# excamera/alfalfa

Measured on AMD Instinct MI355X. Metric: 1080p macroblocks/s decode (bit-exact vs reference), higher is better.
Workload: dtype u8

## Files before the change

### alfalfa_amd/csrc/parse_common.hh

```
#pragma once
#include <stddef.h>
#include <stdint.h>

#include "../../include/alfalfa_amd.h"
#include "vp8_tables.h"

#if defined( __HIPCC__ )
#define AA_HD __host__ __device__
#else
#define AA_HD
#endif

namespace aa {

enum MbMode : uint8_t { DC_PRED, V_PRED, H_PRED, TM_PRED, B_PRED, NEARESTMV, NEARMV, ZEROMV, NEWMV, SPLITMV };
enum BMode : uint8_t { B_DC_PRED, B_TM_PRED, B_VE_PRED, B_HE_PRED, B_LD_PRED, B_RD_PRED, B_VR_PRED, B_VL_PRED,
                       B_HD_PRED, B_HU_PRED, LEFT4X4, ABOVE4X4, ZERO4X4, NEW4X4 };
enum RefFrame : uint8_t { CURRENT_FRAME, LAST_FRAME, GOLDEN_FRAME, ALTREF_FRAME };
enum BlockType { Y_AFTER_Y2 = 0, Y2 = 1, UV = 2, Y_WITHOUT_Y2 = 3 };

constexpr int8_t kKfYModeTree[8] = { -B_PRED, 2, 4, 6, -DC_PRED, -V_PRED, -H_PRED, -TM_PRED };
constexpr int8_t kYModeTree[8] = { -DC_PRED, 2, 4, 6, -V_PRED, -H_PRED, -TM_PRED, -B_PRED };
constexpr int8_t kUvModeTree[6] = { -DC_PRED, 2, -V_PRED, 4, -H_PRED, -TM_PRED };
constexpr int8_t kBModeTree[18] = { -B_DC_PRED, 2, -B_TM_PRED, 4, -B_VE_PRED, 6, 8, 12, -B_HE_PRED, 10,
                                    -B_RD_PRED, -B_VR_PRED, -B_LD_PRED, 14, -B_VL_PRED, 16, -B_HD_PRED, -B_HU_PRED };
constexpr int8_t kSmallMvTree[14] = { 2, 8, 4, 6, -0, -1, -2, -3, 10, 12, -4, -5, -6, -7 };
constexpr int8_t kMvRefTree[8] = { -ZEROMV, 2, -NEARESTMV, 4, -NEARMV, 6, -NEWMV, -SPLITMV };
constexpr int8_t kSubMvRefTree[6] = { -LEFT4X4, 2, -ABOVE4X4, 4, -ZERO4X4, -NEW4X4 };
constexpr int8_t kSplitMvTree[6] = { -3, 2, -2, 4, -0, -1 };
constexpr int8_t kSegmentIdTree[6] = { 2, 4, -0, -1, -2, -3 };

constexpr uint8_t kZigzag[16] = { 0, 1, 4, 8, 5, 2, 3, 6, 9, 12, 13, 10, 7, 11, 14, 15 };
constexpr uint8_t kBand[17] = { 0, 1, 2, 3, 6, 4, 5, 6, 6, 6, 6, 6, 6, 6, 6, 7, 0 };

constexpr uint8_t kSplitLayout[4][16] = { { 0, 0, 0, 0, 0, 0, 0, 0, 1, 1, 1, 1, 1, 1, 1, 1 },
                                          { 0, 0, 1, 1, 0, 0, 1, 1, 0, 0, 1, 1, 0, 0, 1, 1 },
                                          { 0, 0, 1, 1, 0, 0, 1, 1, 2, 2, 3, 3, 2, 2, 3, 3 },
                                          { 0, 1, 2, 3, 4, 5, 6, 7, 8, 9, 10, 11, 12, 13, 14, 15 } };
constexpr uint8_t kSplitFirst[4][16] = { { 0, 8 }, { 0, 2 }, { 0, 2, 8, 10 }, { 0, 1, 2, 3, 4, 5, 6, 7, 8, 9, 10, 11, 12, 13, 14, 15 } };
constexpr uint8_t kSplitCount[4] = { 2, 2, 4, 16 };

struct CoeffProbs { uint8_t coeff_probs[4][8][3][11]; };
struct HeaderParams {
  uint32_t first_off, first_size;
  uint32_t bd_bitpos;
  uint8_t bd_range, bd_active;
  uint8_t key, nparts;
  uint32_t part_off[8], part_size[8];
  uint16_t mbw, mbh;
  uint8_t seg_enabled, seg_update_map, seg_tree_probs[3];
  uint8_t skip_enabled, prob_skip, prob_inter, prob_last, prob_golden;
  uint8_t sign_bias_golden, sign_bias_alt;
  uint8_t loop_filter_level, fadj_enabled;
  int8_t fadj_ref[4], fadj_mode[4];
  int16_t seg_level[4];
  uint8_t y_mode_probs[4], uv_mode_probs[3], mv_probs[2][19];
  uint8_t pad[3];
};
struct FrameParams : CoeffProbs, HeaderParams {};
static_assert( sizeof( FrameParams ) % 4 == 0 && sizeof( HeaderParams ) % 4 == 0 && sizeof( FrameParams ) == sizeof( CoeffProbs ) + sizeof( HeaderParams ),
               "FrameParams / HeaderParams are copied as words" );

struct HeaderTables {
  int8_t kf_y_mode_tree[8], y_mode_tree[8], uv_mode_tree[6], b_mode_tree[18], small_mv_tree[14], mv_ref_tree[8], sub_mv_ref_tree[6], split_mv_tree[6], segment_id_tree[6];
  uint8_t kf_y_mode_probs[4], kf_uv_mode_probs[3], b_mode_probs[9], mv_counts_to_probs[24], split_mv_probs[3], submv_ref_probs[15];
  uint8_t split_layout[4][16], split_first[4][16], split_count[4];
  uint8_t kf_b_mode_probs[900];
  uint8_t pad[2];
};
static_assert( sizeof( HeaderTables ) % 4 == 0, "HeaderTables is copied as words" );
constexpr HeaderTables make_header_tables()
{
  HeaderTables t {};
  for ( int i = 0; i < 8; i++ ) { t.kf_y_mode_tree[i] = kKfYModeTree[i]; t.y_mode_tree[i] = kYModeTree[i]; t.mv_ref_tree[i] = kMvRefTree[i]; }
  for ( int i = 0; i < 6; i++ ) { t.uv_mode_tree[i] = kUvModeTree[i]; t.sub_mv_ref_tree[i] = kSubMvRefTree[i]; t.split_mv_tree[i] = kSplitMvTree[i]; t.segment_id_tree[i] = kSegmentIdTree[i]; }
  for ( int i = 0; i < 18; i++ ) t.b_mode_tree[i] = kBModeTree[i];
  for ( int i = 0; i < 14; i++ ) t.small_mv_tree[i] = kSmallMvTree[i];
  for ( int i = 0; i < 4; i++ ) t.kf_y_mode_probs[i] = k_kf_y_mode_probs[i];
  for ( int i = 0; i < 3; i++ ) { t.kf_uv_mode_probs[i] = k_kf_uv_mode_probs[i]; t.split_mv_probs[i] = k_split_mv_probs[i]; }
  for ( int i = 0; i < 9; i++ ) t.b_mode_probs[i] = k_b_mode_probs[i];
  for ( int i = 0; i < 24; i++ ) t.mv_counts_to_probs[i] = k_mv_counts_to_probs[i];
  for ( int i = 0; i < 15; i++ ) t.submv_ref_probs[i] = k_submv_ref_probs[i];
  for ( int i = 0; i < 4; i++ ) { t.split_count[i] = kSplitCount[i]; for ( int j = 0; j < 16; j++ ) { t.split_layout[i][j] = kSplitLayout[i][j]; t.split_first[i][j] = kSplitFirst[i][j]; } }
  for ( int i = 0; i < 900; i++ ) t.kf_b_mode_probs[i] = k_kf_b_mode_probs[i];
  return t;
}
constexpr HeaderTables kHeaderTables = make_header_tables();



struct BoolState { uint32_t bitpos; uint8_t range, active; };

class BoolReader32
{
  const uint8_t * base_ = nullptr;
  uint32_t pos_ = 0, end_ = 0;
  uint32_t value_ = 0;
  int count_ = 0;
  uint32_t range_ = 255;
  uint32_t cache_ = 0;
  uint32_t cache_n_ = 0;

  AA_HD inline uint32_t next_byte()
  {
    if ( cache_n_ == 0 ) {
      if ( pos_ < end_ ) {
        const uintptr_t a = reinterpret_cast<uintptr_t>( base_ + pos_ );
        const uint32_t skip = static_cast<uint32_t>( a & 3u );
        cache_ = *reinterpret_cast<const uint32_t *>( a - skip ) >> ( 8u * skip );
        cache_n_ = 4u - skip;
      } else { cache_ = 0; cache_n_ = 4u; }
    }
    const uint32_t byte = pos_ < end_ ? ( cache_ & 0xFFu ) : 0u;
    cache_ >>= 8; cache_n_--; pos_++;
    return byte;
  }

public:
  AA_HD BoolReader32() {}
  AA_HD void resume( const uint8_t * base, uint32_t size, const BoolState & st )
  {
    base_ = base; end_ = size; range_ = st.range;
    const uint32_t byte = st.bitpos >> 3, r = st.bitpos & 7;
    pos_ = byte; cache_n_ = 0;
    uint32_t b = 0;
    for ( int k = 0; k < 3; k++ ) b = ( b << 8 ) | next_byte();
    value_ = ( static_cast<uint32_t>( st.active ) << 24 ) | ( ( b << r ) & 0xFFFFFFu );
    count_ = 24 - static_cast<int>( r );
  }
  AA_HD void reset( const uint8_t * base, uint32_t size )
  {
    BoolState st; st.bitpos = 8; st.range = 255; st.active = size ? base[0] : 0;
    resume( base, size, st );
  }
  AA_HD inline int get( const uint32_t prob )
  {
    const uint32_t split = 1 + ( ( ( range_ - 1 ) * prob ) >> 8 );
    if ( count_ < 0 ) {
      value_ |= next_byte() << ( 16 - count_ );
      count_ += 8;
    }
    const uint32_t bigsplit = split << 24;
    int bit;
    uint32_t range;
    if ( value_ >= bigsplit ) { range = range_ - split; value_ -= bigsplit; bit = 1; }
    else { range = split; bit = 0; }
    const int shift = __builtin_clz( range ) - 24;
    range_ = range << shift;
    value_ <<= shift;
    count_ -= shift;
    return bit;
  }
  AA_HD inline int flag() { return get( 128 ); }
  AA_HD inline int literal( int bits ) { int v = 0; while ( bits-- ) v = ( v << 1 ) | get( 128 ); return v; }
  AA_HD inline int tree( const int8_t * nodes, const uint8_t * probs )
  {
    int i = 0;
    while ( ( i = nodes[i + get( probs[i >> 1] )] ) > 0 ) {}
    return -i;
  }
};

struct Mv {
  int16_t x = 0, y = 0;
  AA_HD bool zero() const { return x == 0 && y == 0; }
  AA_HD bool operator==( const Mv & o ) const { return x == o.x && y == o.y; }
};

AA_HD inline int clamp_int( int v, int lo, int hi ) { return v < lo ? lo : ( v > hi ? hi : v ); }

template <class BD>
AA_HD inline int16_t read_mv_component( BD & bd, const uint8_t * p, const HeaderTables & T )
{
  enum { MV_IS_SHORT, SIGN, SHORT, BITS = SHORT + 8 - 1, MV_LONG_BITS = 10 };
  int x = 0;
  if ( bd.get( p[MV_IS_SHORT] ) ) {
    for ( int i = 0; i < 3; i++ ) x += bd.get( p[BITS + i] ) << i;
    for ( int i = MV_LONG_BITS - 1; i > 3; i-- ) x += bd.get( p[BITS + i] ) << i;
    if ( !( x & 0xFFF0 ) || bd.get( p[BITS + 3] ) ) x += 8;
  } else {
    x = bd.tree( T.small_mv_tree, p + SHORT );
  }
  x <<= 1;
  if ( x && bd.get( p[SIGN] ) ) x = -x;
  return static_cast<int16_t>( x );
}

template <class BD>
AA_HD inline Mv read_mv( BD & bd, const HeaderParams & fp, const HeaderTables & T )
{
  Mv m;
  m.y = read_mv_component( bd, fp.mv_probs[0], T );
  m.x = read_mv_component( bd, fp.mv_probs[1], T );
  return m;
}

AA_HD inline Mv clamp_mv( Mv m, unsigned col, unsigned row, unsigned mbw, unsigned mbh )
{
  const int to_left = clamp_int( -( static_cast<int>( col * 16 ) << 3 ) - 128, -32768, 32767 );
  const int to_right = clamp_int( ( static_cast<int>( ( mbw - 1 - col ) * 16 ) << 3 ) + 128, -32768, 32767 );
  const int to_top = clamp_int( -( static_cast<int>( row * 16 ) << 3 ) - 128, -32768, 32767 );
  const int to_bottom = clamp_int( ( static_cast<int>( ( mbh - 1 - row ) * 16 ) << 3 ) + 128, -32768, 32767 );
  m.x = static_cast<int16_t>( clamp_int( m.x, to_left, to_right ) );
  m.y = static_cast<int16_t>( clamp_int( m.y, to_top, to_bottom ) );
  return m;
}

AA_HD inline uint8_t mb_lf_level( const HeaderParams & fp, unsigned segment_id, unsigned ref_frame, unsigned y_mode )
{
  if ( !fp.loop_filter_level ) return 0;
  int level = fp.seg_level[segment_id];
  if ( fp.fadj_enabled ) {
    level += fp.fadj_ref[ref_frame];
    if ( ref_frame == CURRENT_FRAME ) level += ( y_mode == B_PRED ) ? fp.fadj_mode[0] : 0;
    else if ( y_mode == ZEROMV ) level += fp.fadj_mode[1];
    else if ( y_mode == SPLITMV ) level += fp.fadj_mode[3];
    else level += fp.fadj_mode[2];
  }
  return static_cast<uint8_t>( level <= 0 ? 0 : ( level > 63 ? 63 : level ) );
}

AA_HD inline void segment_fixup( const HeaderParams & fp, aa_mb_info & mb, uint8_t & map )
{
  if ( fp.seg_update_map ) map = mb.segment_id;
  else {
    mb.segment_id = map;
    mb.lf_level = mb_lf_level( fp, map, mb.ref_frame, mb.y_mode );
  }
}

AA_HD inline bool mv_flipped( const HeaderParams & fp, unsigned ref_frame )
{
  return ( ref_frame == GOLDEN_FRAME && fp.sign_bias_golden ) || ( ref_frame == ALTREF_FRAME && fp.sign_bias_alt );
}

template <class BD>
AA_HD inline uint8_t parse_mb_header( BD & bd, const HeaderParams & fp, const HeaderTables & T, aa_mb_info * mbs, unsigned mi, unsigned col, unsigned row,
                                      uint8_t * segmap )
{
  const unsigned mbw = fp.mbw, mbh = fp.mbh;
  const bool key = fp.key;
  aa_mb_info & mb = mbs[mi];
  {
    uint32_t * w = reinterpret_cast<uint32_t *>( &mb );
    for ( unsigned k = 0; k < sizeof( aa_mb_info ) / 4; k++ ) w[k] = 0;
  }

  unsigned segment_id = 0;
  if ( fp.seg_enabled ) {
    if ( fp.seg_update_map ) {
      segment_id = static_cast<unsigned>( bd.tree( T.segment_id_tree, fp.seg_tree_probs ) );
      if ( segmap ) segmap[mi] = static_cast<uint8_t>( segment_id );
    } else if ( segmap ) segment_id = segmap[mi];
  }
  mb.segment_id = static_cast<uint8_t>( segment_id );
  const bool skip = fp.skip_enabled ? bd.get( fp.prob_skip ) : false;
  bool inter = false;
  if ( !key ) {
    inter = bd.get( fp.prob_inter );
    if ( inter ) {
      mb.ref_frame = LAST_FRAME;
      if ( bd.get( fp.prob_last ) ) mb.ref_frame = bd.get( fp.prob_golden ) ? ALTREF_FRAME : GOLDEN_FRAME;
    }
  }

  if ( !inter ) {
    mb.y_mode = static_cast<uint8_t>( key ? bd.tree( T.kf_y_mode_tree, T.kf_y_mode_probs ) : bd.tree( T.y_mode_tree, fp.y_mode_probs ) );
    if ( mb.y_mode == B_PRED ) {
      uint8_t bm[16];
      uint8_t above4[4] = { B_DC_PRED, B_DC_PRED, B_DC_PRED, B_DC_PRED }, left4[4] = { B_DC_PRED, B_DC_PRED, B_DC_PRED, B_DC_PRED };
      if ( key ) {
        if ( row > 0 ) for ( int k = 0; k < 4; k++ ) above4[k] = mbs[mi - mbw].u.b_mode[12 + k];
        if ( col > 0 ) for ( int k = 0; k < 4; k++ ) left4[k] = mbs[mi - 1].u.b_mode[4 * k + 3];
      }
#if defined( __HIP_DEVICE_COMPILE__ )
#pragma unroll
#endif
      for ( int b = 0; b < 16; b++ ) {
        if ( key ) {
          const int above_mode = b >= 4 ? bm[b - 4] : above4[b];
          const int left_mode = ( b & 3 ) ? bm[b - 1] : left4[b >> 2];
          bm[b] = static_cast<uint8_t>( bd.tree( T.b_mode_tree, T.kf_b_mode_probs + ( above_mode * 10 + left_mode ) * 9 ) );
        } else {
          bm[b] = static_cast<uint8_t>( bd.tree( T.b_mode_tree, T.b_mode_probs ) );
        }
      }
      for ( int b = 0; b < 16; b++ ) mb.u.b_mode[b] = bm[b];
    } else {
      constexpr uint8_t kImplied[4] = { B_DC_PRED, B_VE_PRED, B_HE_PRED, B_TM_PRED };
      const uint8_t m = kImplied[mb.y_mode];
      for ( int b = 0; b < 16; b++ ) mb.u.b_mode[b] = m;
    }
    mb.uv_mode = static_cast<uint8_t>( key ? bd.tree( T.uv_mode_tree, T.kf_uv_mode_probs ) : bd.tree( T.uv_mode_tree, fp.uv_mode_probs ) );
  } else {
    mb.flags |= AA_MB_INTER;
    uint8_t score[4] = { 0, 0, 0, 0 };
    Mv cand[4];
    int idx = 0, split_score = 0;
    const bool my_flip = mv_flipped( fp, mb.ref_frame );
    auto consider = [&]( unsigned ni, int weight ) {
      const aa_mb_info & nb = mbs[ni];
      if ( !( nb.flags & AA_MB_INTER ) ) return;
      Mv mv; mv.x = nb.u.mv[15][0]; mv.y = nb.u.mv[15][1];
      if ( mv_flipped( fp, nb.ref_frame ) != my_flip ) { mv.x = static_cast<int16_t>( -mv.x ); mv.y = static_cast<int16_t>( -mv.y ); }
      if ( mv.zero() ) score[0] += weight;
      else {
        if ( !( mv == cand[idx] ) ) cand[++idx] = mv;
        score[idx] += weight;
      }
      if ( nb.y_mode == SPLITMV ) split_score += weight;
    };
    if ( row > 0 ) consider( mi - mbw, 2 );
    if ( col > 0 ) consider( mi - 1, 2 );
    if ( row > 0 && col > 0 ) consider( mi - mbw - 1, 1 );
    if ( score[3] && cand[idx] == cand[1] ) score[1] += score[3];
    if ( score[2] > score[1] ) {
      const uint8_t ts = score[1]; score[1] = score[2]; score[2] = ts;
      const Mv tm = cand[1]; cand[1] = cand[2]; cand[2] = tm;
    }
    if ( score[1] >= score[0] ) cand[0] = cand[1];
    const uint8_t mode_probs[4] = { T.mv_counts_to_probs[score[0] * 4 + 0], T.mv_counts_to_probs[score[1] * 4 + 1],
                                    T.mv_counts_to_probs[score[2] * 4 + 2], T.mv_counts_to_probs[split_score * 4 + 3] };
    mb.y_mode = static_cast<uint8_t>( bd.tree( T.mv_ref_tree, mode_probs ) );
    Mv base;
    switch ( mb.y_mode ) {
    case NEARESTMV: base = clamp_mv( cand[1], col, row, mbw, mbh ); break;
    case NEARMV: base = clamp_mv( cand[2], col, row, mbw, mbh ); break;
    case ZEROMV: break;
    case NEWMV: {
      const Mv delta = read_mv( bd, fp, T );
      const Mv best = clamp_mv( cand[0], col, row, mbw, mbh );
      base.x = static_cast<int16_t>( delta.x + best.x ); base.y = static_cast<int16_t>( delta.y + best.y );
      break; }
    default: {
      mb.split_partition = static_cast<uint8_t>( bd.tree( T.split_mv_tree, T.split_mv_probs ) );
      const Mv best = clamp_mv( cand[0], col, row, mbw, mbh );
      const uint8_t * layout = T.split_layout[mb.split_partition];
      for ( int part = 0; part < T.split_count[mb.split_partition]; part++ ) {
        const int b = T.split_first[mb.split_partition][part];
        Mv lmv, amv;
        if ( b & 3 ) { lmv.x = mb.u.mv[b - 1][0]; lmv.y = mb.u.mv[b - 1][1]; }
        else if ( col > 0 && ( mbs[mi - 1].flags & AA_MB_INTER ) ) { lmv.x = mbs[mi - 1].u.mv[b + 3][0]; lmv.y = mbs[mi - 1].u.mv[b + 3][1]; }
        if ( b >= 4 ) { amv.x = mb.u.mv[b - 4][0]; amv.y = mb.u.mv[b - 4][1]; }
        else if ( row > 0 && ( mbs[mi - mbw].flags & AA_MB_INTER ) ) { amv.x = mbs[mi - mbw].u.mv[b + 12][0]; amv.y = mbs[mi - mbw].u.mv[b + 12][1]; }
        int ctx = 0;
        if ( lmv == amv ) ctx = lmv.zero() ? 4 : 3;
        else if ( amv.zero() ) ctx = 2;
        else if ( lmv.zero() ) ctx = 1;
        Mv m;
        switch ( bd.tree( T.sub_mv_ref_tree, T.submv_ref_probs + ctx * 3 ) ) {
        case LEFT4X4: m = lmv; break;
        case ABOVE4X4: m = amv; break;
        case ZERO4X4: break;
        default: { const Mv d = read_mv( bd, fp, T ); m.x = static_cast<int16_t>( d.x + best.x ); m.y = static_cast<int16_t>( d.y + best.y ); break; }
        }
        for ( int k = 0; k < 16; k++ ) if ( layout[k] == part ) { mb.u.mv[k][0] = m.x; mb.u.mv[k][1] = m.y; }
      }
      break; }
    }
    if ( mb.y_mode != SPLITMV ) for ( int k = 0; k < 16; k++ ) { mb.u.mv[k][0] = base.x; mb.u.mv[k][1] = base.y; }
  }

  if ( !( mb.y_mode == B_PRED || mb.y_mode == SPLITMV ) ) mb.flags |= AA_MB_HAS_Y2;
  if ( skip ) mb.flags |= AA_MB_SKIP;
  mb.lf_level = mb_lf_level( fp, segment_id, mb.ref_frame, mb.y_mode );
  return mb.flags;
}

}
```

### alfalfa_amd/csrc/parse_kernels.hip

```cpp
#include <hip/hip_runtime.h>

#include <algorithm>

#include "device_types.h"
#include "tok_fsm.hh"
#include "coeff_pack.hh"

#ifndef AA_WORKER_PRIO
#define AA_WORKER_PRIO 3
#endif

namespace {

using aa::ParseJob;

__global__ __launch_bounds__( 64 ) void k_parse_mb_headers( const ParseJob * jobs, const uint32_t * order, int n, int lanes )
{
  __builtin_amdgcn_s_setprio( 2 );

  __shared__ aa::HeaderTables s_tables;
  __shared__ aa::HeaderParams s_params[16];
  const int lane = threadIdx.x;
  for ( uint32_t k = lane; k < sizeof( aa::HeaderTables ) / 4; k += 64 ) reinterpret_cast<uint32_t *>( &s_tables )[k] = reinterpret_cast<const uint32_t *>( &aa::kHeaderTables )[k];
  const int slot = blockIdx.x * lanes + lane;
  const bool mine = lane < lanes && lane < 16 && slot < n;
  const ParseJob * Jp = mine ? &jobs[order[slot]] : nullptr;
  if ( Jp ) {
    const uint32_t * src = reinterpret_cast<const uint32_t *>( static_cast<const aa::HeaderParams *>( &Jp->fp ) );
    for ( uint32_t k = 0; k < sizeof( aa::HeaderParams ) / 4; k++ ) reinterpret_cast<uint32_t *>( &s_params[lane] )[k] = src[k];
  }
  __syncthreads();
  if ( !Jp ) return;
  const ParseJob & J = *Jp;
  if ( J.nmb == 0 ) return;
  const aa::HeaderParams & fp = s_params[lane];
  const aa::HeaderTables & T = s_tables;
  aa::BoolReader32 bd;
  aa::BoolState st; st.bitpos = fp.bd_bitpos; st.range = fp.bd_range; st.active = fp.bd_active;
  bd.resume( J.data + fp.first_off, fp.first_size, st );
  const unsigned mbw = fp.mbw, mbh = fp.mbh;
  const unsigned words_per_row = ( mbw + 63 ) / 64;
  uint32_t intra = 0, split = 0;
  unsigned mi = 0;
  const uint32_t mp_stride = J.mp_stride, mp_base = J.flags_padded, nparts = fp.nparts;
  for ( unsigned row = 0; row < mbh; row++ ) {
    unsigned long long word = 0;
    const uint32_t mp_row = mp_stride ? mp_base + ( row % nparts ) * mp_stride + ( row / nparts ) * mbw : 0u;
    for ( unsigned col = 0; col < mbw; col++, mi++ ) {
      const uint8_t flags = aa::parse_mb_header( bd, fp, T, J.mbs, mi, col, row, static_cast<uint8_t *>( nullptr ) );
      J.mbflags[mi] = flags;
      if ( mp_stride ) J.mbflags[mp_row + col] = flags;
      if ( !( flags & AA_MB_INTER ) ) { intra++; word |= 1ull << ( col & 63 ); }
      else if ( J.mbs[mi].y_mode == aa::SPLITMV ) split = 1;
      if ( ( col & 63 ) == 63 || col + 1 == mbw ) { J.intra_rows[row * words_per_row + ( col >> 6 )] = word; word = 0; }
    }
  }
  J.summary->num_intra_mbs = intra;
  J.summary->has_split = split;
}

__global__ __launch_bounds__( 256 ) void k_segment_fixup( const ParseJob * jobs, const aa_seg_stream * streams, const uint32_t * order )
{
  const aa_seg_stream s = streams[blockIdx.x];
  for ( uint32_t k = 0; k < s.count; k++ ) {
    const uint32_t o = order[s.first + k];
    const ParseJob & J = jobs[o & 0x7FFFFFFFu];
    if ( !J.fp.seg_enabled || J.nmb == 0 ) continue;
    if ( o >> 31 ) {
      for ( uint32_t mi = threadIdx.x; mi < J.nmb; mi += blockDim.x ) s.map[mi] = 3;
      __syncthreads();
    }
    for ( uint32_t mi = threadIdx.x; mi < J.nmb; mi += blockDim.x ) aa::segment_fixup( J.fp, J.mbs[mi], s.map[mi] );
    __syncthreads();
  }
}

struct WorkerArgs {
  aa::TokQueue * q;
  unsigned long long * slots;
  aa::Heap heap;
  uint32_t * exited;
  const uint32_t * retire;
  uint32_t gen;
  uint32_t spread;
  unsigned long long * prof;
  unsigned long long linger_ticks;
  int lanes;
  uint32_t lane_bytes;
  uint32_t mp_hint;
  uint32_t * cu_slots;
  uint32_t cu_cap;
  int16_t * sink;
};

__device__ inline uint32_t queue_take( aa::TokQueue * q, uint32_t want, uint32_t spread, uint32_t * base )
{
  uint32_t h = AA_AT_LOAD( &q->head );
  for ( uint32_t tries = 0; ; tries++ ) {
    const uint32_t avail = AA_AT_LOAD( &q->publish ) - h;
    if ( static_cast<int32_t>( avail ) <= 0 ) return 0;
    const uint32_t share = ( avail + spread - 1u ) / spread;
    const uint32_t n = want < share ? want : share;
    uint32_t expect = h;
    if ( __hip_atomic_compare_exchange_strong( &q->head, &expect, h + n, __ATOMIC_RELAXED, __ATOMIC_RELAXED, __HIP_MEMORY_SCOPE_AGENT ) ) { *base = h; return n; }
    h = expect;
    const uint32_t r = ( blockIdx.x * 2654435761u + tries * 40503u ) >> 27;
    for ( uint32_t k = 0; k <= ( r & ( tries < 4 ? 3u : tries < 8 ? 15u : 31u ) ); k++ ) __builtin_amdgcn_s_sleep( 16 );
    if ( tries > 2048 ) h = AA_AT_LOAD( &q->head );
  }
}

__device__ inline int nth_set_bit( unsigned long long mask, uint32_t n )
{
  for ( uint32_t k = 0; k < n; k++ ) mask &= mask - 1ull;
  return __ffsll( static_cast<long long>( mask ) ) - 1;
}

template <bool PK, bool MP>
__global__ __launch_bounds__( 64 ) void k_token_workers( const WorkerArgs a )
{
  extern __shared__ __attribute__( ( aligned( 16 ) ) ) uint8_t smem[];
  const int lane = threadIdx.x;
#if AA_WORKER_PRIO
  __builtin_amdgcn_s_setprio( AA_WORKER_PRIO );
#endif
  uint32_t cu_slot = 0;
  if ( a.cu_slots ) {
    const uint32_t hw = __builtin_amdgcn_s_getreg( 4 | ( 8 << 6 ) | ( 7 << 11 ) ), xcc = __builtin_amdgcn_s_getreg( 20 | ( 0 << 6 ) | ( 3 << 11 ) );
    cu_slot = ( ( xcc & 15u ) << 8 ) | ( hw & 255u );
    uint32_t before = 0;
    if ( lane == 0 ) before = AA_AT_ADD( &a.cu_slots[cu_slot], 1u );
    before = __shfl( before, 0 );
    if ( before >= a.cu_cap ) {
      if ( lane == 0 ) { AA_AT_ADD( &a.cu_slots[cu_slot], 0xFFFFFFFFu ); AA_AT_ADD( &a.cu_slots[AA_CU_SLOTS - 1], 1u ); AA_AT_ADD( a.exited, 1u ); }
      return;
    }
  }
  for ( uint32_t k = lane; k < aa::tok::kTablesBytes / 4; k += 64 ) reinterpret_cast<uint32_t *>( smem )[k] = aa::tok::table_word( k );
  __syncthreads();
  aa::tok::Lane L;
  aa::tok::Frame F {};
  const bool is_lane = lane < a.lanes;
  aa::tok::init_lane( L, aa::tok::ring_addr( is_lane ? lane : 0 ), aa::tok::slice_addr( is_lane ? lane : 0, a.lanes, a.lane_bytes ),
                      (AA_GLOBAL int16_t *) ( a.sink + ( blockIdx.x & 63u ) * 32u + ( lane & 31 ) ) );
  aa::tok::preload( L, smem );
  uint32_t backoff = 0;
  unsigned long long idle_since = 0;
  uint32_t looks = 0;
  bool retiring = false;
  aa::tok::PeriodProf pp { 0, 0, 0 };
  unsigned long long p_look = 0, p_topup = 0, p_period = 0, p_lanes = 0, p_periods = 0;
  const bool profiling = a.prof != nullptr;
  const auto prof_flush = [&]() {
    __hip_atomic_fetch_add( &a.prof[0], pp.pass_ticks, __ATOMIC_RELAXED, __HIP_MEMORY_SCOPE_AGENT );
    __hip_atomic_fetch_add( &a.prof[1], pp.passes, __ATOMIC_RELAXED, __HIP_MEMORY_SCOPE_AGENT );
    __hip_atomic_fetch_add( &a.prof[2], pp.steps, __ATOMIC_RELAXED, __HIP_MEMORY_SCOPE_AGENT );
    __hip_atomic_fetch_add( &a.prof[3], p_look, __ATOMIC_RELAXED, __HIP_MEMORY_SCOPE_AGENT );
    __hip_atomic_fetch_add( &a.prof[4], p_topup, __ATOMIC_RELAXED, __HIP_MEMORY_SCOPE_AGENT );
    __hip_atomic_fetch_add( &a.prof[5], p_period, __ATOMIC_RELAXED, __HIP_MEMORY_SCOPE_AGENT );
    __hip_atomic_fetch_add( &a.prof[6], p_lanes, __ATOMIC_RELAXED, __HIP_MEMORY_SCOPE_AGENT );
    __hip_atomic_fetch_add( &a.prof[7], p_periods, __ATOMIC_RELAXED, __HIP_MEMORY_SCOPE_AGENT );
  };
  for ( ;; ) {
    const unsigned long long t_a = profiling ? wall_clock64() : 0ull;
    const bool idle = is_lane && L.rec == aa::tok::R_DONE;
    const unsigned long long idle_mask = __ballot( idle );
    bool looked = false;
    if ( idle_mask && !retiring ) {
      if ( backoff ) backoff--;
      else {
        looked = true;
        const int first = __ffsll( static_cast<long long>( idle_mask ) ) - 1;
        uint32_t base = 0, got = 0;
        if ( lane == first ) {
          if ( ( looks++ & 7u ) == 0 && __hip_atomic_load( a.retire, __ATOMIC_RELAXED, __HIP_MEMORY_SCOPE_SYSTEM ) >= a.gen ) got = 0xFFFFFFFFu;
          else {
            uint32_t want = static_cast<uint32_t>( __popcll( idle_mask ) );
            if constexpr ( MP ) want = want / a.mp_hint > 1u ? want / a.mp_hint : 1u;
            got = queue_take( a.q, want, a.spread, &base );
          }
        }
        base = __shfl( base, first ); got = __shfl( got, first );
        if ( got == 0xFFFFFFFFu ) { retiring = true; got = 0; }
        const uint32_t rank = static_cast<uint32_t>( __popcll( idle_mask & ( ( 1ull << lane ) - 1ull ) ) );
        const bool mine = idle && rank < got;
        if ( got ) {
          __builtin_amdgcn_fence( __ATOMIC_ACQUIRE, "agent" );
          const aa::ParseJob * job = nullptr;
          if ( mine ) job = reinterpret_cast<const aa::ParseJob *>( AA_AT_LOAD( &a.slots[( base + rank ) & a.q->mask] ) );
          if constexpr ( MP ) {
            const uint32_t n_idle = static_cast<uint32_t>( __popcll( idle_mask ) );
            const int my_parts = mine ? static_cast<int>( job->nmb && job->mp_stride ? job->fp.nparts : 1u ) : 1;
            const aa::tok::MpDeal d = aa::tok::mp_deal( n_idle, got, rank, [&]( uint32_t t ) {
              return static_cast<uint32_t>( __shfl( my_parts, nth_set_bit( idle_mask, t ) ) ); } );
            const long long jp = __shfl( static_cast<long long>( reinterpret_cast<uintptr_t>( job ) ), nth_set_bit( idle_mask, d.ticket ) );
            if ( idle && d.any ) {
              const aa::ParseJob * my_job = reinterpret_cast<const aa::ParseJob *>( static_cast<uintptr_t>( jp ) );
              if ( d.n > 1u ) {
                const int owner_lane = nth_set_bit( idle_mask, d.start + aa::tok::mp_owner_partition( my_job ) );
                F = aa::tok::frame_of_partition( my_job, d.part, aa::tok::slice_addr( owner_lane, a.lanes, a.lane_bytes ) );
              } else F = aa::tok::frame_of( my_job );
              if ( my_job->nmb == 0 ) { L.rec = aa::tok::R_DONE; aa::tok::preload( L, smem ); }
              else aa::tok::begin_frame<MP>( L, smem, L.base, F );
            }
          } else if ( mine ) {
            F = aa::tok::frame_of( job );
            if ( F.nmb == 0 ) { L.rec = aa::tok::R_DONE; aa::tok::preload( L, smem ); }
            else aa::tok::begin_frame<MP>( L, smem, L.base, F );
          }
// ... 218 lines not shown
```

Before: 127.2 million.

## Restructure MB header parser to carry neighbours in registers and prefetch bitstream

Measured after the change: 103.2 million. 0.811x the previous value.

```diff
diff --git a/alfalfa_amd/csrc/parse_common.hh b/alfalfa_amd/csrc/parse_common.hh
--- a/alfalfa_amd/csrc/parse_common.hh
+++ b/alfalfa_amd/csrc/parse_common.hh
@@ -9,6 +9,18 @@
 #define AA_HD __host__ __device__
 #else
 #define AA_HD
+#endif
+#if defined( __HIP_DEVICE_COMPILE__ )
+#define AA_INLINE __attribute__( ( always_inline ) ) inline
+#else
+#define AA_INLINE inline
+#endif
+#if !defined( AA_GLOBAL )
+#if defined( __HIP_DEVICE_COMPILE__ )
+#define AA_GLOBAL __attribute__( ( address_space( 1 ) ) )
+#else
+#define AA_GLOBAL
+#endif
 #endif
 
 namespace aa {
@@ -100,16 +112,22 @@
   uint32_t range_ = 255;
   uint32_t cache_ = 0;
   uint32_t cache_n_ = 0;
-
-  AA_HD inline uint32_t next_byte()
+  uint32_t ahead_ = 0;
+
+  AA_HD AA_INLINE void look_ahead( uint32_t off )
+  {
+    if ( off < end_ ) ahead_ = *reinterpret_cast<const AA_GLOBAL uint32_t *>( reinterpret_cast<uintptr_t>( base_ + off ) );
+  }
+  AA_HD AA_INLINE uint32_t next_byte()
   {
     if ( cache_n_ == 0 ) {
-      if ( pos_ < end_ ) {
-        const uintptr_t a = reinterpret_cast<uintptr_t>( base_ + pos_ );
-        const uint32_t skip = static_cast<uint32_t>( a & 3u );
-        cache_ = *reinterpret_cast<const uint32_t *>( a - skip ) >> ( 8u * skip );
-        cache_n_ = 4u - skip;
-      } else { cache_ = 0; cache_n_ = 4u; }
+#if defined( __HIP_DEVICE_COMPILE__ )
+      asm volatile( "v_mov_b32 %0, %1" : "=v"( cache_ ) : "v"( ahead_ ) );
+#else
+      cache_ = ahead_;
+#endif
+      cache_n_ = 4u;
+      look_ahead( pos_ + 4u );
     }
     const uint32_t byte = pos_ < end_ ? ( cache_ & 0xFFu ) : 0u;
     cache_ >>= 8; cache_n_--; pos_++;
@@ -122,7 +140,13 @@
   {
     base_ = base; end_ = size; range_ = st.range;
     const uint32_t byte = st.bitpos >> 3, r = st.bitpos & 7;
-    pos_ = byte; cache_n_ = 0;
+    pos_ = byte; cache_ = 0; cache_n_ = 4u;
+    if ( pos_ < end_ ) {
+      const uint32_t skip = static_cast<uint32_t>( reinterpret_cast<uintptr_t>( base_ + pos_ ) & 3u );
+      cache_ = *reinterpret_cast<const AA_GLOBAL uint32_t *>( reinterpret_cast<uintptr_t>( base_ + pos_ - skip ) ) >> ( 8u * skip );
+      cache_n_ = 4u - skip;
+    }
+    ahead_ = 0; look_ahead( pos_ + cache_n_ );
     uint32_t b = 0;
     for ( int k = 0; k < 3; k++ ) b = ( b << 8 ) | next_byte();
     value_ = ( static_cast<uint32_t>( st.active ) << 24 ) | ( ( b << r ) & 0xFFFFFFu );
@@ -133,9 +157,9 @@
     BoolState st; st.bitpos = 8; st.range = 255; st.active = size ? base[0] : 0;
     resume( base, size, st );
   }
-  AA_HD inline int get( const uint32_t prob )
+  AA_HD AA_INLINE int get( const uint32_t prob )
   {
-    const uint32_t split = 1 + ( ( ( range_ - 1 ) * prob ) >> 8 );
+    const uint32_t split = 1 + ( ( ( ( range_ - 1 ) & 0xFFu ) * ( prob & 0xFFu ) ) >> 8 );
     if ( count_ < 0 ) {
       value_ |= next_byte() << ( 16 - count_ );
       count_ += 8;
@@ -153,10 +177,13 @@
   }
   AA_HD inline int flag() { return get( 128 ); }
   AA_HD inline int literal( int bits ) { int v = 0; while ( bits-- ) v = ( v << 1 ) | get( 128 ); return v; }
-  AA_HD inline int tree( const int8_t * nodes, const uint8_t * probs )
+  AA_HD AA_INLINE int tree( const int8_t * nodes, const uint8_t * probs )
   {
     int i = 0;
-    while ( ( i = nodes[i + get( probs[i >> 1] )] ) > 0 ) {}
+    do {
+      const int zero = nodes[i], one = nodes[i + 1];
+      i = get( probs[i >> 1] ) ? one : zero;
+    } while ( i > 0 );
     return -i;
   }
 };
@@ -167,10 +194,10 @@
   AA_HD bool operator==( const Mv & o ) const { return x == o.x && y == o.y; }
 };
 
-AA_HD inline int clamp_int( int v, int lo, int hi ) { return v < lo ? lo : ( v > hi ? hi : v ); }
+AA_HD AA_INLINE int clamp_int( int v, int lo, int hi ) { return v < lo ? lo : ( v > hi ? hi : v ); }
 
 template <class BD>
-AA_HD inline int16_t read_mv_component( BD & bd, const uint8_t * p, const HeaderTables & T )
+AA_HD AA_INLINE int16_t read_mv_component( BD & bd, const uint8_t * p, const HeaderTables & T )
 {
   enum { MV_IS_SHORT, SIGN, SHORT, BITS = SHORT + 8 - 1, MV_LONG_BITS = 10 };
   int x = 0;
@@ -187,7 +214,7 @@
 }
 
 template <class BD>
-AA_HD inline Mv read_mv( BD & bd, const HeaderParams & fp, const HeaderTables & T )
+AA_HD AA_INLINE Mv read_mv( BD & bd, const HeaderParams & fp, const HeaderTables & T )
 {
   Mv m;
   m.y = read_mv_component( bd, fp.mv_probs[0], T );
@@ -195,7 +222,7 @@
   return m;
 }
 
-AA_HD inline Mv clamp_mv( Mv m, unsigned col, unsigned row, unsigned mbw, unsigned mbh )
+AA_HD AA_INLINE Mv clamp_mv( Mv m, unsigned col, unsigned row, unsigned mbw, unsigned mbh )
 {
   const int to_left = clamp_int( -( static_cast<int>( col * 16 ) << 3 ) - 128, -32768, 32767 );
   const int to_right = clamp_int( ( static_cast<int>( ( mbw - 1 - col ) * 16 ) << 3 ) + 128, -32768, 32767 );
@@ -206,7 +233,7 @@
   return m;
 }
 
-AA_HD inline uint8_t mb_lf_level( const HeaderParams & fp, unsigned segment_id, unsigned ref_frame, unsigned y_mode )
+AA_HD AA_INLINE uint8_t mb_lf_level( const HeaderParams & fp, unsigned segment_id, unsigned ref_frame, unsigned y_mode )
 {
   if ( !fp.loop_filter_level ) return 0;
   int level = fp.seg_level[segment_id];
@@ -229,142 +256,291 @@
   }
 }
 
-AA_HD inline bool mv_flipped( const HeaderParams & fp, unsigned ref_frame )
+AA_HD AA_INLINE bool mv_flipped( const HeaderParams & fp, unsigned ref_frame )
 {
   return ( ref_frame == GOLDEN_FRAME && fp.sign_bias_golden ) || ( ref_frame == ALTREF_FRAME && fp.sign_bias_alt );
+}
+
+
+struct MbRecord { uint32_t w[20]; };
+static_assert( sizeof( MbRecord ) == sizeof( aa_mb_info ) && sizeof( aa_mb_info ) == 80, "a record is twenty words" );
+
+struct MbNeighbour { uint32_t inter = 0, ref_frame = 0, y_mode = 0, bm = 0, mv[4] = { 0, 0, 0, 0 }; };
+
+AA_HD AA_INLINE MbNeighbour neighbour_above( uint32_t w0, uint32_t w1, uint32_t w7, uint32_t w16, uint32_t w17, uint32_t w18, uint32_t w19 )
+{
+  MbNeighbour n;
+  n.inter = ( w1 & AA_MB_INTER ) ? 1u : 0u; n.ref_frame = ( w0 >> 16 ) & 0xFFu; n.y_mode = w0 & 0xFFu;
+  n.bm = w7;
+  n.mv[0] = w16; n.mv[1] = w17; n.mv[2] = w18; n.mv[3] = w19;
+  return n;
+}
+AA_HD AA_INLINE MbNeighbour neighbour_above( const MbRecord & r ) { return neighbour_above( r.w[0], r.w[1], r.w[7], r.w[16], r.w[17], r.w[18], r.w[19] ); }
+AA_HD AA_INLINE MbNeighbour neighbour_left( const MbRecord & r )
+{
+  MbNeighbour n;
+  n.inter = ( r.w[1] & AA_MB_INTER ) ? 1u : 0u; n.ref_frame = ( r.w[0] >> 16 ) & 0xFFu; n.y_mode = r.w[0] & 0xFFu;
+  n.bm = ( r.w[4] >> 24 ) | ( ( r.w[5] >> 24 ) << 8 ) | ( ( r.w[6] >> 24 ) << 16 ) | ( r.w[7] & 0xFF000000u );
+  n.mv[0] = r.w[7]; n.mv[1] = r.w[11]; n.mv[2] = r.w[15]; n.mv[3] = r.w[19];
+  return n;
+}
+
+AA_HD AA_INLINE uint32_t pack_mv( int x, int y ) { return ( static_cast<uint32_t>( x ) & 0xFFFFu ) | ( static_cast<uint32_t>( y ) << 16 ); }
+AA_HD AA_INLINE Mv unpack_mv( uint32_t v ) { Mv m; m.x = static_cast<int16_t>( v & 0xFFFFu ); m.y = static_cast<int16_t>( v >> 16 ); return m; }
+AA_HD AA_INLINE uint32_t negate_mv( uint32_t v ) { const Mv m = unpack_mv( v ); return pack_mv( -m.x, -m.y ); }
+AA_HD AA_INLINE uint32_t select4( uint32_t a0, uint32_t a1, uint32_t a2, uint32_t a3, unsigned i ) { return i == 0 ? a0 : ( i == 1 ? a1 : ( i == 2 ? a2 : a3 ) ); }
+
+struct Census { unsigned s0 = 0, s1 = 0, s2 = 0, s3 = 0, split = 0, idx = 0; uint32_t c1 = 0, c2 = 0, c3 = 0; };
+AA_HD AA_INLINE Census census_consider( Census c, const HeaderParams & fp, const MbNeighbour & nb, const unsigned weight, const bool my_flip )
+{
+  if ( !nb.inter ) return c;
+  uint32_t mv = nb.mv[3];
+  if ( mv_flipped( fp, nb.ref_frame ) != my_flip ) mv = negate_mv( mv );
+  if ( mv == 0 ) c.s0 += weight;
+  else {
+    const bool fresh = mv != select4( 0u, c.c1, c.c2, c.c3, c.idx );
+    const unsigned idx = c.idx + ( fresh ? 1u : 0u );
+    c.c1 = ( fresh && idx == 1 ) ? mv : c.c1; c.c2 = ( fresh && idx == 2 ) ? mv : c.c2; c.c3 = ( fresh && idx == 3 ) ? mv : c.c3;
+    c.s1 += idx == 1 ? weight : 0u; c.s2 += idx == 2 ? weight : 0u; c.s3 += idx == 3 ? weight : 0u;
+    c.idx = idx;
+  }
+  if ( nb.y_mode == SPLITMV ) c.split += weight;
+  return c;
+}
+
+template <class BD>
+AA_HD AA_INLINE MbRecord parse_mb_header_core( BD & bd, const HeaderParams & fp, const HeaderTables & T, const unsigned col, const unsigned row,
+                                               const MbNeighbour left, const MbNeighbour above, const MbNeighbour above_left, const unsigned seg_inherited )
+{
+  const unsigned mbw = fp.mbw, mbh = fp.mbh;
+  const bool key = fp.key;
+
+  unsigned segment_id = 0;
+  if ( fp.seg_enabled ) segment_id = fp.seg_update_map ? static_cast<unsigned>( bd.tree( T.segment_id_tree, fp.seg_tree_probs ) ) : seg_inherited;
+  const bool skip = fp.skip_enabled ? bd.get( fp.prob_skip ) : false;
+  bool inter = false;
+  unsigned ref_frame = CURRENT_FRAME;
+  if ( !key ) {
+    inter = bd.get( fp.prob_inter );
+    if ( inter ) {
+      ref_frame = LAST_FRAME;
+      if ( bd.get( fp.prob_last ) ) ref_frame = bd.get( fp.prob_golden ) ? ALTREF_FRAME : GOLDEN_FRAME;
+    }
+  }
+
+  unsigned y_mode, uv_mode = 0, split_partition = 0;
+  uint32_t u[16];
+#if defined( __HIP_DEVICE_COMPILE__ )
+#pragma unroll
+#endif
+  for ( int k = 0; k < 16; k++ ) u[k] = 0;
+
+  if ( !inter ) {
+    y_mode = static_cast<unsigned>( bd.tree( key ? T.kf_y_mode_tree : T.y_mode_tree, key ? T.kf_y_mode_probs : fp.y_mode_probs ) );
+    if ( y_mode == B_PRED ) {
+      unsigned long long modes = 0;
+      const uint32_t above4 = ( key && row > 0 ) ? above.bm : 0u, left4 = ( key && col > 0 ) ? left.bm : 0u;
+      const auto context = [&]( unsigned b ) {
+        if ( !key ) return T.b_mode_probs;
+        const unsigned above_mode = b >= 4 ? static_cast<unsigned>( modes >> 48 ) & 15u : ( above4 >> ( 8u * ( b & 3u ) ) ) & 0xFFu;
+        const unsigned left_mode = ( b & 3u ) ? static_cast<unsigned>( modes >> 60 ) : ( left4 >> ( 8u * ( b >> 2 ) ) ) & 0xFFu;
+        return T.kf_b_mode_probs + ( above_mode * 10u + left_mode ) * 9u;
+      };
+      const uint8_t * probs = context( 0 );
+      unsigned b = 0;
+      int i = 0;
+      for ( ;; ) {
+        const int zero = T.b_mode_tree[i], one = T.b_mode_tree[i + 1];
+        i = bd.get( probs[i >> 1] ) ? one : zero;
+        if ( i > 0 ) continue;
+        modes = ( modes >> 4 ) | ( static_cast<unsigned long long>( -i ) << 60 );
+        if ( ++b == 16 ) break;
+        probs = context( b );
+        i = 0;
+      }
+#if defined( __HIP_DEVICE_COMPILE__ )
+#pragma unroll
+#endif
+      for ( int k = 0; k < 4; k++ ) {
+        const uint32_t n = static_cast<uint32_t>( modes >> ( 16 * k ) ) & 0xFFFFu;
+        u[k] = ( n & 0xFu ) | ( ( n & 0xF0u ) << 4 ) | ( ( n & 0xF00u ) << 8 ) | ( ( n & 0xF000u ) << 12 );
+      }
+    } else {
+      const uint32_t m = select4( B_DC_PRED, B_VE_PRED, B_HE_PRED, B_TM_PRED, y_mode ) * 0x01010101u;
+      u[0] = m; u[1] = m; u[2] = m; u[3] = m;
+    }
+    uv_mode = static_cast<unsigned>( bd.tree( T.uv_mode_tree, key ? T.kf_uv_mode_probs : fp.uv_mode_probs ) );
+  } else {
+    Census cs;
+    const bool my_flip = mv_flipped( fp, ref_frame );
+    if ( row > 0 ) cs = census_consider( cs, fp, above, 2, my_flip );
+    if ( col > 0 ) cs = census_consider( cs, fp, left, 2, my_flip );
+    if ( row > 0 && col > 0 ) cs = census_consider( cs, fp, above_left, 1, my_flip );
+    unsigned s0 = cs.s0, s1 = cs.s1, s2 = cs.s2;
+    const unsigned split_score = cs.split;
+    uint32_t c1 = cs.c1, c2 = cs.c2;
+    if ( cs.s3 && select4( 0u, cs.c1, cs.c2, cs.c3, cs.idx ) == c1 ) s1 += cs.s3;
+    if ( s2 > s1 ) {
+      const unsigned ts = s1; s1 = s2; s2 = ts;
+      const uint32_t tm = c1; c1 = c2; c2 = tm;
+    }
+    const uint32_t c0 = s1 >= s0 ? c1 : 0u;
+    const uint32_t mode_probs = static_cast<uint32_t>( T.mv_counts_to_probs[s0 * 4 + 0] ) | ( static_cast<uint32_t>( T.mv_counts_to_probs[s1 * 4 + 1] ) << 8 )
+                                | ( static_cast<uint32_t>( T.mv_counts_to_probs[s2 * 4 + 2] ) << 16 ) | ( static_cast<uint32_t>( T.mv_counts_to_probs[split_score * 4 + 3] ) << 24 );
+    unsigned link = 0;
+#if defined( __HIP_DEVICE_COMPILE__ )
+#pragma unroll 1
+#endif
+    for ( ; link < 4; link++ ) if ( !bd.get( ( mode_probs >> ( 8u * link ) ) & 0xFFu ) ) break;
+    y_mode = link == 0 ? ZEROMV : ( link == 1 ? NEARESTMV : ( link == 2 ? NEARMV : ( link == 3 ? NEWMV : SPLITMV ) ) );
+    const Mv best = clamp_mv( unpack_mv( y_mode == NEARESTMV ? c1 : ( y_mode == NEARMV ? c2 : c0 ) ), col, row, mbw, mbh );
+    uint32_t base = 0;
+    if ( y_mode == NEARESTMV || y_mode == NEARMV ) base = pack_mv( best.x, best.y );
+    else if ( y_mode == NEWMV ) {
+      const Mv delta = read_mv( bd, fp, T );
+      base = pack_mv( static_cast<int16_t>( delta.x + best.x ), static_cast<int16_t>( delta.y + best.y ) );
+    }
+    if ( y_mode == SPLITMV ) {
+      split_partition = static_cast<unsigned>( bd.tree( T.split_mv_tree, T.split_mv_probs ) );
+      const uint8_t * layout = T.split_layout[split_partition];
+      const uint8_t * first = T.split_first[split_partition];
+      const bool left_inter = col > 0 && left.inter, above_inter = row > 0 && above.inter;
+#if defined( __HIP_DEVICE_COMPILE__ )
+#pragma unroll 1
+#endif
+      for ( unsigned b = 0; b < 16; b++ ) {
+        const unsigned part = layout[b];
+        uint32_t m;
+        if ( first[part] == b ) {
+          uint32_t lmv = 0, amv = 0;
+          if ( b & 3u ) lmv = u[15];
+          else if ( left_inter ) lmv = select4( left.mv[0], left.mv[1], left.mv[2], left.mv[3], b >> 2 );
+          if ( b >= 4 ) amv = u[12];
+          else if ( above_inter ) amv = select4( above.mv[0], above.mv[1], above.mv[2], above.mv[3], b );
+          unsigned ctx = 0;
+          if ( lmv == amv ) ctx = lmv == 0 ? 4 : 3;
+          else if ( amv == 0 ) ctx = 2;
+          else if ( lmv == 0 ) ctx = 1;
+          const int sub = bd.tree( T.sub_mv_ref_tree, T.submv_ref_probs + ctx * 3 );
+          if ( sub == LEFT4X4 ) m = lmv;
+          else if ( sub == ABOVE4X4 ) m = amv;
+          else if ( sub == ZERO4X4 ) m = 0;
+          else { const Mv d = read_mv( bd, fp, T ); m = pack_mv( static_cast<int16_t>( d.x + best.x ), static_cast<int16_t>( d.y + best.y ) ); }
+        } else m = ( ( b & 3u ) && layout[b - 1] == part ) ? u[15] : u[12];
+#if defined( __HIP_DEVICE_COMPILE__ )
+#pragma unroll
+#endif
+        for ( int k = 0; k < 15; k++ ) u[k] = u[k + 1];
+        u[15] = m;
+      }
+    } else {
+#if defined( __HIP_DEVICE_COMPILE__ )
+#pragma unroll
+#endif
+      for ( int k = 0; k < 16; k++ ) u[k] = base;
+    }
+  }
+
+  unsigned flags = inter ? AA_MB_INTER : 0u;
+  if ( !( y_mode == B_PRED || y_mode == SPLITMV ) ) flags |= AA_MB_HAS_Y2;
+  if ( skip ) flags |= AA_MB_SKIP;
+  const unsigned lf_level = mb_lf_level( fp, segment_id, ref_frame, y_mode );
+  MbRecord r;
+  r.w[0] = y_mode | ( uv_mode << 8 ) | ( ref_frame << 16 ) | ( segment_id << 24 );
+  r.w[1] = flags | ( lf_level << 8 ) | ( split_partition << 16 );
+  r.w[2] = 0; r.w[3] = 0;
+#if defined( __HIP_DEVICE_COMPILE__ )
+#pragma unroll
+#endif
+  for ( int k = 0; k < 16; k++ ) r.w[4 + k] = u[k];
+  return r;
 }
 
 template <class BD>
 AA_HD inline uint8_t parse_mb_header( BD & bd, const HeaderParams & fp, const HeaderTables & T, aa_mb_info * mbs, unsigned mi, unsigned col, unsigned row,
                                       uint8_t * segmap )
 {
-  const unsigned mbw = fp.mbw, mbh = fp.mbh;
-  const bool key = fp.key;
-  aa_mb_info & mb = mbs[mi];
-  {
-    uint32_t * w = reinterpret_cast<uint32_t *>( &mb );
-    for ( unsigned k = 0; k < sizeof( aa_mb_info ) / 4; k++ ) w[k] = 0;
-  }
-
-  unsigned segment_id = 0;
-  if ( fp.seg_enabled ) {
-    if ( fp.seg_update_map ) {
-      segment_id = static_cast<unsigned>( bd.tree( T.segment_id_tree, fp.seg_tree_probs ) );
-      if ( segmap ) segmap[mi] = static_cast<uint8_t>( segment_id );
-    } else if ( segmap ) segment_id = segmap[mi];
-  }
-  mb.segment_id = static_cast<uint8_t>( segment_id );
-  const bool skip = fp.skip_enabled ? bd.get( fp.prob_skip ) : false;
-  bool inter = false;
-  if ( !key ) {
-    inter = bd.get( fp.prob_inter );
-    if ( inter ) {
-      mb.ref_frame = LAST_FRAME;
-      if ( bd.get( fp.prob_last ) ) mb.ref_frame = bd.get( fp.prob_golden ) ? ALTREF_FRAME : GOLDEN_FRAME;
-    }
-  }
-
-  if ( !inter ) {
-    mb.y_mode = static_cast<uint8_t>( key ? bd.tree( T.kf_y_mode_tree, T.kf_y_mode_probs ) : bd.tree( T.y_mode_tree, fp.y_mode_probs ) );
-    if ( mb.y_mode == B_PRED ) {
-      uint8_t bm[16];
-      uint8_t above4[4] = { B_DC_PRED, B_DC_PRED, B_DC_PRED, B_DC_PRED }, left4[4] = { B_DC_PRED, B_DC_PRED, B_DC_PRED, B_DC_PRED };
-      if ( key ) {
-        if ( row > 0 ) for ( int k = 0; k < 4; k++ ) above4[k] = mbs[mi - mbw].u.b_mode[12 + k];
-        if ( col > 0 ) for ( int k = 0; k < 4; k++ ) left4[k] = mbs[mi - 1].u.b_mode[4 * k + 3];
-      }
+  const unsigned mbw = fp.mbw;
+  const auto record = [&]( unsigned ni ) { MbRecord r; __builtin_memcpy( r.w, &mbs[ni], sizeof r.w ); return r; };
+  MbNeighbour left, above, above_left;
+  if ( col > 0 ) left = neighbour_left( record( mi - 1 ) );
+  if ( row > 0 ) above = neighbour_above( record( mi - mbw ) );
+  if ( row > 0 && col > 0 ) above_left = neighbour_above( record( mi - mbw - 1 ) );
+  const bool inherits = fp.seg_enabled && !fp.seg_update_map && segmap;
+  const MbRecord r = parse_mb_header_core( bd, fp, T, col, row, left, above, above_left, inherits ? segmap[mi] : 0u );
+  if ( fp.seg_enabled && fp.seg_update_map && segmap ) segmap[mi] = static_cast<uint8_t>( r.w[0] >> 24 );
+  __builtin_memcpy( &mbs[mi], r.w, sizeof r.w );
+  return static_cast<uint8_t>( r.w[1] );
+}
+
+struct alignas( 8 ) Words2 { uint32_t x, y; };
+struct alignas( 16 ) Words4 { uint32_t x, y, z, w; };
+AA_HD AA_INLINE Words2 load_words2( const AA_GLOBAL void * p )
+{
+#if defined( __HIP_DEVICE_COMPILE__ )
+  return *static_cast<const AA_GLOBAL Words2 *>( p );
+#else
+  Words2 v; __builtin_memcpy( &v, p, sizeof v ); return v;
+#endif
+}
+AA_HD AA_INLINE Words4 load_words4( const AA_GLOBAL void * p )
+{
+#if defined( __HIP_DEVICE_COMPILE__ )
+  return *static_cast<const AA_GLOBAL Words4 *>( p );
+#else
+  Words4 v; __builtin_memcpy( &v, p, sizeof v ); return v;
+#endif
+}
+AA_HD AA_INLINE void store_words4( AA_GLOBAL void * p, uint32_t x, uint32_t y, uint32_t z, uint32_t w )
+{
+  Words4 v; v.x = x; v.y = y; v.z = z; v.w = w;
+#if defined( __HIP_DEVICE_COMPILE__ )
+  *static_cast<AA_GLOBAL Words4 *>( p ) = v;
+#else
+  __builtin_memcpy( p, &v, sizeof v );
+#endif
+}
+
+struct HeaderLoopOut {
+  AA_GLOBAL aa_mb_info * mbs;
+  AA_GLOBAL uint8_t * mbflags;
+  AA_GLOBAL unsigned long long * intra_rows;
+  uint32_t mp_stride, mp_base;
+};
+
+template <class BD>
+AA_HD AA_INLINE void parse_mb_headers_loop( BD & bd, const HeaderParams & fp, const HeaderTables & T, const HeaderLoopOut o, uint32_t & intra_out, uint32_t & split_out )
+{
+  const unsigned mbw = fp.mbw, mbh = fp.mbh, nparts = fp.nparts;
+  const unsigned words_per_row = ( mbw + 63 ) / 64;
+  uint32_t intra = 0, split = 0;
+  unsigned mi = 0;
+  MbNeighbour left, above, above_left;
+  for ( unsigned row = 0; row < mbh; row++ ) {
+    unsigned long long word = 0;
+    const uint32_t mp_row = o.mp_stride ? o.mp_base + ( row % nparts ) * o.mp_stride + ( row / nparts ) * mbw : 0u;
+    for ( unsigned col = 0; col < mbw; col++, mi++ ) {
+      const AA_GLOBAL uint32_t * nw = reinterpret_cast<const AA_GLOBAL uint32_t *>( o.mbs + ( mi + 1 >= mbw ? mi + 1 - mbw : 0u ) );
+      const Words2 n01 = load_words2( nw );
+      const Words4 n4 = load_words4( nw + 4 ), n16 = load_words4( nw + 16 );
+      const MbRecord r = parse_mb_header_core( bd, fp, T, col, row, left, above, above_left, 0u );
+      AA_GLOBAL uint32_t * out = reinterpret_cast<AA_GLOBAL uint32_t *>( o.mbs + mi );
 #if defined( __HIP_DEVICE_COMPILE__ )
 #pragma unroll
 #endif
-      for ( int b = 0; b < 16; b++ ) {
-        if ( key ) {
-          const int above_mode = b >= 4 ? bm[b - 4] : above4[b];
-          const int left_mode = ( b & 3 ) ? bm[b - 1] : left4[b >> 2];
-          bm[b] = static_cast<uint8_t>( bd.tree( T.b_mode_tree, T.kf_b_mode_probs + ( above_mode * 10 + left_mode ) * 9 ) );
-        } else {
-          bm[b] = static_cast<uint8_t>( bd.tree( T.b_mode_tree, T.b_mode_probs ) );
-        }
-      }
-      for ( int b = 0; b < 16; b++ ) mb.u.b_mode[b] = bm[b];
-    } else {
-      constexpr uint8_t kImplied[4] = { B_DC_PRED, B_VE_PRED, B_HE_PRED, B_TM_PRED };
-      const uint8_t m = kImplied[mb.y_mode];
-      for ( int b = 0; b < 16; b++ ) mb.u.b_mode[b] = m;
-    }
-    mb.uv_mode = static_cast<uint8_t>( key ? bd.tree( T.uv_mode_tree, T.kf_uv_mode_probs ) : bd.tree( T.uv_mode_tree, fp.uv_mode_probs ) );
-  } else {
-    mb.flags |= AA_MB_INTER;
-    uint8_t score[4] = { 0, 0, 0, 0 };
-    Mv cand[4];
-    int idx = 0, split_score = 0;
-    const bool my_flip = mv_flipped( fp, mb.ref_frame );
-    auto consider = [&]( unsigned ni, int weight ) {
-      const aa_mb_info & nb = mbs[ni];
-      if ( !( nb.flags & AA_MB_INTER ) ) return;
-      Mv mv; mv.x = nb.u.mv[15][0]; mv.y = nb.u.mv[15][1];
-      if ( mv_flipped( fp, nb.ref_frame ) != my_flip ) { mv.x = static_cast<int16_t>( -mv.x ); mv.y = static_cast<int16_t>( -mv.y ); }
-      if ( mv.zero() ) score[0] += weight;
-      else {
-        if ( !( mv == cand[idx] ) ) cand[++idx] = mv;
-        score[idx] += weight;
-      }
-      if ( nb.y_mode == SPLITMV ) split_score += weight;
-    };
-    if ( row > 0 ) consider( mi - mbw, 2 );
-    if ( col > 0 ) consider( mi - 1, 2 );
-    if ( row > 0 && col > 0 ) consider( mi - mbw - 1, 1 );
-    if ( score[3] && cand[idx] == cand[1] ) score[1] += score[3];
-    if ( score[2] > score[1] ) {
-      const uint8_t ts = score[1]; score[1] = score[2]; score[2] = ts;
-      const Mv tm = cand[1]; cand[1] = cand[2]; cand[2] = tm;
-    }
-    if ( score[1] >= score[0] ) cand[0] = cand[1];
-    const uint8_t mode_probs[4] = { T.mv_counts_to_probs[score[0] * 4 + 0], T.mv_counts_to_probs[score[1] * 4 + 1],
-                                    T.mv_counts_to_probs[score[2] * 4 + 2], T.mv_counts_to_probs[split_score * 4 + 3] };
-    mb.y_mode = static_cast<uint8_t>( bd.tree( T.mv_ref_tree, mode_probs ) );
-    Mv base;
-    switch ( mb.y_mode ) {
-    case NEARESTMV: base = clamp_mv( cand[1], col, row, mbw, mbh ); break;
-    case NEARMV: base = clamp_mv( cand[2], col, row, mbw, mbh ); break;
-    case ZEROMV: break;
-    case NEWMV: {
-      const Mv delta = read_mv( bd, fp, T );
-      const Mv best = clamp_mv( cand[0], col, row, mbw, mbh );
-      base.x = static_cast<int16_t>( delta.x + best.x ); base.y = static_cast<int16_t>( delta.y + best.y );
-      break; }
-    default: {
-      mb.split_partition = static_cast<uint8_t>( bd.tree( T.split_mv_tree, T.split_mv_probs ) );
-      const Mv best = clamp_mv( cand[0], col, row, mbw, mbh );
-      const uint8_t * layout = T.split_layout[mb.split_partition];
-      for ( int part = 0; part < T.split_count[mb.split_partition]; part++ ) {
-        const int b = T.split_first[mb.split_partition][part];
-        Mv lmv, amv;
-        if ( b & 3 ) { lmv.x = mb.u.mv[b - 1][0]; lmv.y = mb.u.mv[b - 1][1]; }
-        else if ( col > 0 && ( mbs[mi - 1].flags & AA_MB_INTER ) ) { lmv.x = mbs[mi - 1].u.mv[b + 3][0]; lmv.y = mbs[mi - 1].u.mv[b + 3][1]; }
-        if ( b >= 4 ) { amv.x = mb.u.mv[b - 4][0]; amv.y = mb.u.mv[b - 4][1]; }
-        else if ( row > 0 && ( mbs[mi - mbw].flags & AA_MB_INTER ) ) { amv.x = mbs[mi - mbw].u.mv[b + 12][0]; amv.y = mbs[mi - mbw].u.mv[b + 12][1]; }
-        int ctx = 0;
-        if ( lmv == amv ) ctx = lmv.zero() ? 4 : 3;
-        else if ( amv.zero() ) ctx = 2;
-        else if ( lmv.zero() ) ctx = 1;
-        Mv m;
-        switch ( bd.tree( T.sub_mv_ref_tree, T.submv_ref_probs + ctx * 3 ) ) {
-        case LEFT4X4: m = lmv; break;
-        case ABOVE4X4: m = amv; break;
-        case ZERO4X4: break;
-        default: { const Mv d = read_mv( bd, fp, T ); m.x = static_cast<int16_t>( d.x + best.x ); m.y = static_cast<int16_t>( d.y + best.y ); break; }
-        }
-        for ( int k = 0; k < 16; k++ ) if ( layout[k] == part ) { mb.u.mv[k][0] = m.x; mb.u.mv[k][1] = m.y; }
-      }
-      break; }
-    }
-    if ( mb.y_mode != SPLITMV ) for ( int k = 0; k < 16; k++ ) { mb.u.mv[k][0] = base.x; mb.u.mv[k][1] = base.y; }
-  }
-
-  if ( !( mb.y_mode == B_PRED || mb.y_mode == SPLITMV ) ) mb.flags |= AA_MB_HAS_Y2;
-  if ( skip ) mb.flags |= AA_MB_SKIP;
-  mb.lf_level = mb_lf_level( fp, segment_id, mb.ref_frame, mb.y_mode );
-  return mb.flags;
-}
-
-}
+      for ( int k = 0; k < 5; k++ ) store_words4( out + 4 * k, r.w[4 * k], r.w[4 * k + 1], r.w[4 * k + 2], r.w[4 * k + 3] );
+      const uint8_t flags = static_cast<uint8_t>( r.w[1] );
+      o.mbflags[mi] = flags;
+      if ( o.mp_stride ) o.mbflags[mp_row + col] = flags;
+      if ( !( flags & AA_MB_INTER ) ) { intra++; word |= 1ull << ( col & 63 ); }
+      else if ( ( r.w[0] & 0xFFu ) == SPLITMV ) split = 1;
+      if ( ( col & 63 ) == 63 || col + 1 == mbw ) { o.intra_rows[row * words_per_row + ( col >> 6 )] = word; word = 0; }
+      above_left = above;
+      left = neighbour_left( r );
+      above = mbw == 1 ? neighbour_above( r ) : neighbour_above( n01.x, n01.y, n4.w, n16.x, n16.y, n16.z, n16.w );
+    }
+  }
+  intra_out = intra; split_out = split;
+}
+
+}
diff --git a/alfalfa_amd/csrc/parse_kernels.hip b/alfalfa_amd/csrc/parse_kernels.hip
--- a/alfalfa_amd/csrc/parse_kernels.hip
+++ b/alfalfa_amd/csrc/parse_kernels.hip
@@ -38,23 +38,11 @@
   aa::BoolReader32 bd;
   aa::BoolState st; st.bitpos = fp.bd_bitpos; st.range = fp.bd_range; st.active = fp.bd_active;
   bd.resume( J.data + fp.first_off, fp.first_size, st );
-  const unsigned mbw = fp.mbw, mbh = fp.mbh;
-  const unsigned words_per_row = ( mbw + 63 ) / 64;
+  aa::HeaderLoopOut o;
+  o.mbs = (AA_GLOBAL aa_mb_info *) J.mbs; o.mbflags = (AA_GLOBAL uint8_t *) J.mbflags; o.intra_rows = (AA_GLOBAL unsigned long long *) J.intra_rows;
+  o.mp_stride = J.mp_stride; o.mp_base = J.flags_padded;
   uint32_t intra = 0, split = 0;
-  unsigned mi = 0;
-  const uint32_t mp_stride = J.mp_stride, mp_base = J.flags_padded, nparts = fp.nparts;
-  for ( unsigned row = 0; row < mbh; row++ ) {
-    unsigned long long word = 0;
-    const uint32_t mp_row = mp_stride ? mp_base + ( row % nparts ) * mp_stride + ( row / nparts ) * mbw : 0u;
-    for ( unsigned col = 0; col < mbw; col++, mi++ ) {
-      const uint8_t flags = aa::parse_mb_header( bd, fp, T, J.mbs, mi, col, row, static_cast<uint8_t *>( nullptr ) );
-      J.mbflags[mi] = flags;
-      if ( mp_stride ) J.mbflags[mp_row + col] = flags;
-      if ( !( flags & AA_MB_INTER ) ) { intra++; word |= 1ull << ( col & 63 ); }
-      else if ( J.mbs[mi].y_mode == aa::SPLITMV ) split = 1;
-      if ( ( col & 63 ) == 63 || col + 1 == mbw ) { J.intra_rows[row * words_per_row + ( col >> 6 )] = word; word = 0; }
-    }
-  }
+  aa::parse_mb_headers_loop( bd, fp, T, o, intra, split );
   J.summary->num_intra_mbs = intra;
   J.summary->has_split = split;
 }
```
